# InternetMaximalism/plonky2_bn254

Measured on AMD Instinct MI355X. Metric: G1 scalar-mul STARK proofs/sec (256-bit scalars), higher is better.
Workload: dtype u64 (Goldilocks p = 2^64-2^32+1; BN254 Fq as 10x26-bit Montgomery limbs); 1 GPU; configs[1]: batch of 1024 G1 scalar-muls on 1 GPU per step = 8 proofs x 128 instances, 2^16 rows, W=781, standard_fast_config; instances_per_proof=128, steps_in_flight=4, parallelism=1 GPU, no collective

## Files before the change

### include/bn254_stark.h

```cpp
#ifndef BN254_STARK_H
#define BN254_STARK_H

#include <stddef.h>
#include <stdint.h>

#ifdef __cplusplus
extern "C" {
#endif

#define BN254S_ABI_VERSION 1

enum {
  BN254S_OK = 0,
  BN254S_E_INVALID_ARG = -1,
  BN254S_E_HIP = -2,
  BN254S_E_OOM = -3,
  BN254S_E_INVALID_POINT = -4,
  BN254S_E_UNSUPPORTED = -5,
  BN254S_E_TRANSCRIPT = -6,
  BN254S_E_INTERNAL = -7,
  BN254S_E_VERIFY = -8
};

typedef struct bn254s_ctx bn254s_ctx;
// ... 133 lines not shown
                       const uint64_t* offset, size_t n, size_t per_proof, uint64_t* outputs_out, bn254s_proof** proofs_out);
int bn254s_commit_values(bn254s_ctx* ctx, const uint64_t* values, size_t ncols, uint64_t* coeffs, uint64_t* lde,
                         uint64_t* cap);
int bn254s_bench_ntt(bn254s_ctx* ctx, size_t ncols, int iters, float* ms);
int bn254s_bench_ntt_clock(bn254s_ctx* ctx, size_t ncols, int iters, float* ms, float* mhz, float* mhz_min);
int bn254s_bench_issue(bn254s_ctx* ctx, float* ns_per_issue, float* mhz);
int bn254s_bench_copy(bn254s_ctx* ctx, size_t words, int iters);
int bn254s_bench_leafhash(bn254s_ctx* ctx, size_t ncols, int log_leaves, int iters, float* ms);
int bn254s_poseidon_permute(bn254s_ctx* ctx, uint64_t* states, size_t n);
int bn254s_selftest_field(bn254s_ctx* ctx, const uint64_t* a, const uint64_t* b, size_t n, uint64_t* out);
int bn254s_selftest_poseidon(bn254s_ctx* ctx, int variant, uint64_t* states, size_t n);
int bn254s_selftest_leaf_hash(bn254s_ctx* ctx, const uint64_t* data, size_t ncols, int log_leaves, int kernel, int chunk_cols,
                              uint64_t* digests);
int bn254s_selftest_fq_inv(bn254s_ctx* ctx, const uint64_t* x, size_t n, uint64_t* out);
int bn254s_selftest_fq(bn254s_ctx* ctx, int group, const uint64_t* in, size_t n, uint64_t* out);
int bn254s_generate_trace(bn254s_ctx* ctx, int kind, const uint64_t* scalars, const uint64_t* x, const uint64_t* offset,
                          size_t n, uint32_t min_rows_log2, uint64_t* trace_out, uint64_t* outputs);
int bn254s_g1_generate_trace(bn254s_ctx* ctx, const uint64_t* scalars, const uint64_t* x, const uint64_t* offset,
                             size_t n, uint32_t min_rows_log2, uint64_t* trace_out, uint64_t* outputs);

#ifdef __cplusplus
}
#endif
#endif
```

### plonky2_bn254_amd/csrc/aux.hip

```cpp
#include "aux.h"

static constexpr int LOGUP_CHUNK = 30;

__global__ __launch_bounds__(256) void k_logup_helpers(const u64* __restrict__ trace, size_t N, int rc_begin, int n_rc,
                                                       u64 beta0, u64 beta1, u64* __restrict__ aux, int helpers_per_ch,
                                                       u64* __restrict__ psum, int nchunks) {
  const size_t i = (size_t)blockIdx.x * blockDim.x + threadIdx.x;
  if (i >= N) return;
  const int chunk = blockIdx.y, ch = blockIdx.z;
  const u64 beta = ch ? beta1 : beta0;
  const int k0 = chunk * LOGUP_CHUNK;
  const int cnt = min(LOGUP_CHUNK, helpers_per_ch - k0);
  const u64* col = trace + (size_t)(rc_begin + 2 * k0) * N + i;
  u64 prod[LOGUP_CHUNK], pre[LOGUP_CHUNK];
  u64 acc = 1;
#pragma unroll
  for (int j = 0; j < LOGUP_CHUNK; j++) {
    if (j < cnt) {
      const u64 a = gl_add(col[(size_t)(2 * j) * N], beta);
      const bool two = 2 * (k0 + j) + 1 < n_rc;
      prod[j] = two ? gl_mul(a, gl_add(col[(size_t)(2 * j + 1) * N], beta)) : a;
      pre[j] = acc;
      acc = gl_mul(acc, prod[j]);
    }
  }
  u64 inv = gl_inv(acc);
  u64 sum = 0;
  const u64 beta2 = gl_dbl(beta);
  u64* out = aux + (size_t)ch * (helpers_per_ch + 1) * N + i;
#pragma unroll
  for (int j = LOGUP_CHUNK - 1; j >= 0; j--) {
    if (j < cnt) {
      u64 h = gl_mul(inv, pre[j]);
      inv = gl_mul(inv, prod[j]);
      if (2 * (k0 + j) + 1 < n_rc) h = gl_mul(h, gl_add(gl_add(col[(size_t)(2 * j) * N], col[(size_t)(2 * j + 1) * N]), beta2));
      out[(size_t)(k0 + j) * N] = h;
      sum = gl_add(sum, h);
    }
  }
  psum[(size_t)(ch * nchunks + chunk) * N + i] = sum;
}

__global__ __launch_bounds__(256) void k_logup_terms(const u64* __restrict__ trace, size_t N, int table_col, int freq_col,
                                                     u64 beta0, u64 beta1, const u64* __restrict__ psum, int nchunks,
                                                     u64* __restrict__ terms) {
  const size_t i = (size_t)blockIdx.x * blockDim.x + threadIdx.x;
  if (i >= N) return;
  const int ch = blockIdx.y;
  const u64 beta = ch ? beta1 : beta0;
  u64 s = 0;
  for (int c = 0; c < nchunks; c++) s = gl_add(s, psum[(size_t)(ch * nchunks + c) * N + i]);
  u64 t = gl_inv(gl_add(beta, trace[(size_t)table_col * N + i]));
  s = gl_sub(s, gl_mul(trace[(size_t)freq_col * N + i], t));
  terms[(size_t)ch * N + i] = s;
}

__global__ __launch_bounds__(1024) void k_scan(const u64* __restrict__ in, size_t in_stride, u64* __restrict__ out,
                                               size_t out_stride, size_t N, int mode) {
  LATENCY_KERNEL_PRIO();
  __shared__ u64 part[1024];
  const int t = threadIdx.x;
  const u64* src = in + (size_t)blockIdx.x * in_stride;
  u64* dst = out + (size_t)blockIdx.x * out_stride;
  const size_t per = N / 1024;
  auto idx = [&](size_t q) { return mode ? N - 1 - q : q; };
  size_t q0 = (size_t)t * per;
  u64 s = 0;
  for (size_t q = 0; q < per; q++) s = gl_add(s, src[idx(q0 + q)]);
  part[t] = s;
  __syncthreads();
  for (int off = 1; off < 1024; off <<= 1) {
    u64 v = t >= off ? part[t - off] : 0;
    __syncthreads();
    part[t] = gl_add(part[t], v);
    __syncthreads();
  }
  u64 run = t ? part[t - 1] : 0;
  for (size_t q = 0; q < per; q++) {
    u64 x = src[idx(q0 + q)];
    if (mode == 0) {
      dst[idx(q0 + q)] = run;
      run = gl_add(run, x);
    } else {
      run = gl_add(run, x);
      dst[idx(q0 + q)] = run;
    }
// ... 14 lines not shown
      int start = spec.col_start[ctl][m], nb = spec.col_bits[ctl][m];
      u64 v = 0;
      for (int b = nb - 1; b >= 0; b--) v = gl_add(gl_dbl(v), trace[(size_t)(start + b) * N + i]);
      a0 = gl_add(gl_mul(a0, beta0), v);
      a1 = gl_add(gl_mul(a1, beta1), v);
    }
    t0 = gl_inv(gl_add(a0, gamma0));
    t1 = gl_inv(gl_add(a1, gamma1));
  } else if (f != 0) {
    atomicCAS(err, 0, BN254S_E_INTERNAL);
  }
  terms[(size_t)(ctl * 2 + 0) * N + i] = t0;
  terms[(size_t)(ctl * 2 + 1) * N + i] = t1;
}

size_t aux_scratch_words(const StarkShape& sh, size_t N) {
  int nchunks = (sh.n_helpers() + LOGUP_CHUNK - 1) / LOGUP_CHUNK;
  return (size_t)(2 * nchunks + 2 + 2 * sh.n_ctl) * N;
}

void aux_build(const StarkShape& sh, const u64* d_trace, size_t N, const u64 betas[2], const u64 gammas[2], u64* d_aux,
               u64* d_scratch, int* d_err, hipStream_t st) {
  const int n_rc = sh.n_rc(), m = sh.n_helpers();
  const int nchunks = (m + LOGUP_CHUNK - 1) / LOGUP_CHUNK;
  u64* psum = d_scratch;
  u64* terms = psum + (size_t)2 * nchunks * N;
  u64* cterms = terms + 2 * N;
  dim3 g1((unsigned)((N + 255) / 256), nchunks, 2);
  k_logup_helpers<<<g1, 256, 0, st>>>(d_trace, N, sh.rc_begin, n_rc, betas[0], betas[1], d_aux, m, psum, nchunks);
  dim3 g2((unsigned)((N + 255) / 256), 2);
  k_logup_terms<<<g2, 256, 0, st>>>(d_trace, N, sh.table_col, sh.freq_col, betas[0], betas[1], psum, nchunks, terms);
  k_scan<<<2, 1024, 0, st>>>(terms, N, d_aux + (size_t)m * N, (size_t)(m + 1) * N, N, 0);
  dim3 g3((unsigned)((N + 255) / 256), sh.n_ctl);
  k_ctl_terms<<<g3, 256, 0, st>>>(d_trace, N, sh.ctl, betas[0], gammas[0], betas[1], gammas[1], cterms, d_err);
  k_scan<<<2 * sh.n_ctl, 1024, 0, st>>>(cterms, N, d_aux + (size_t)2 * (m + 1) * N, N, N, 1);
}

void aux_module_warm() {
  hipFuncAttributes a;
  (void)hipFuncGetAttributes(&a, reinterpret_cast<const void*>(&k_logup_terms));
}
```

### plonky2_bn254_amd/csrc/capi.hip

```cpp
#include <algorithm>
#include <cstring>
#include "ctx.h"
#include "merkle.h"
#include "trace_g1.h"
#include "fq_selftest.h"
#include "poseidon_dev.h"

void ntt_module_warm();
void merkle_module_warm();
void aux_module_warm();
void fri_module_warm();
void quotient_g1_module_warm();
void quotient_g2fq_module_warm();
void trace_g1_module_warm();
void trace_g2fq_module_warm();
void prover_module_warm();

extern "C" {

int bn254s_abi_version(void) { return BN254S_ABI_VERSION; }

void bn254s_params_default(bn254s_params* p) {
  p->struct_size = sizeof(bn254s_params);
  p->security_bits = 100;
// ... 448 lines not shown

int bn254s_selftest_fq_inv(bn254s_ctx* c, const uint64_t* x, size_t n, uint64_t* out) {
  if (!c || !x || !out) return BN254S_E_INVALID_ARG;
  if (n == 0) return BN254S_OK;
  HIP_TRY(c, hipSetDevice(c->device));
  u64* d = c->words("fi.io", 12 * n);
  if (!d) return BN254S_E_OOM;
  HIP_TRY(c, hipMemcpyAsync(d, x, 32 * n, hipMemcpyHostToDevice, c->stream));
  launch_fq_inv_selftest(d, d + 4 * n, n, c->stream);
  HIP_TRY(c, hipGetLastError());
  HIP_TRY(c, hipMemcpyAsync(out, d + 4 * n, 64 * n, hipMemcpyDeviceToHost, c->stream));
  HIP_TRY(c, hipStreamSynchronize(c->stream));
  return BN254S_OK;
}

static bool selftest_fq_below_p(const uint64_t* w) {
  static const uint64_t P[4] = {0x3c208c16d87cfd47ULL, 0x97816a916871ca8dULL, 0xb85045b68181585dULL, 0x30644e72e131a029ULL};
  for (int j = 3; j >= 0; j--)
    if (w[j] != P[j]) return w[j] < P[j];
  return false;
}
int bn254s_selftest_fq(bn254s_ctx* c, int group, const uint64_t* in, size_t n, uint64_t* out) {
  if (!c || !in || !out || group < 0 || group >= FQ_SELFTEST_GROUPS) return BN254S_E_INVALID_ARG;
  if (n == 0) return BN254S_OK;
  const size_t wi = (size_t)FQ_SELFTEST_IN[group], wo = (size_t)FQ_SELFTEST_OUT[group];
  auto is_zero = [](const uint64_t* w, int words) {
    uint64_t o = 0;
    for (int k = 0; k < words; k++) o |= w[k];
    return o == 0;
  };
// ... 21 lines not shown
```

### plonky2_bn254_amd/csrc/fri.h

```cpp
#pragma once
#include "quotient_common.h"

__host__ __device__ inline size_t merkle_level_offset_dev(int log_leaves, int level) {
  return ((size_t)2 << log_leaves) - ((size_t)2 << (log_leaves - level));
}

static constexpr size_t FRI_OPENING_ZQ_WORDS = 2 * 256 * 4, FRI_OPENING_TABLE_WORDS = 2 * FRI_OPENING_ZQ_WORDS;
void fri_opening_tables(unsigned log_r, gl2 zeta, gl2 zeta_next, u64* d_tables, hipStream_t st);
void fri_openings(const u64* d_coeffs, size_t N, unsigned log_r, int npolys, const u64* d_tables, u64* d_out, hipStream_t st);

void fri_combine(const StarkShape& sh, const u64* d_tl, const u64* d_al, const u64* d_ql, const u64* d_apow, const u64* d_xs,
                 gl2 zeta, gl2 zeta_next, gl2 r0, gl2 r1, gl2 r2, gl2 alpha, size_t M2, u64* d_out, hipStream_t st);

void fri_combine_coeffs(const StarkShape& sh, const u64* d_tcoef, const u64* d_acoef, const u64* d_qcoef, const u64* d_apow, size_t N,
                        u64* d_comb, hipStream_t st);
void fri_combine_final(const StarkShape& sh, const u64* d_comb_lde, const u64* d_xs, gl2 zeta, gl2 zeta_next, gl2 r0, gl2 r1, gl2 r2,
                       gl2 alpha, size_t M2, u64* d_out, hipStream_t st);
void fri_extract_window(const u64* d_lde, size_t M2, unsigned log_n, int h, size_t k0, size_t rows, int ncols, u64* d_out, hipStream_t st);
void fri_gather_rows(const u64* d_lde, size_t M2, int ncols, const u32* d_indices, int nq, u64* d_out, hipStream_t st);

void fri_fold(const u64* d_in, u64* d_out, unsigned log_m, u64 shift, gl2 beta, u64 inv16, hipStream_t st);

void fri_pow_launch(const u64 state[12], int pos, u64 base, unsigned pow_bits, size_t count, unsigned long long* d_result,
                    hipStream_t st);

static constexpr int FRI_MAX_LAYERS = 8;
struct QueryGatherArgs {
// ... 15 lines not shown
```

### plonky2_bn254_amd/csrc/fri.hip

```cpp
#include "fri.h"
#include "poseidon_dev.h"

static constexpr int OPEN_Q = (int)(65536 / 256);

__global__ __launch_bounds__(256) void k_opening_tables(gl2 z0r, gl2 z1r, u64* __restrict__ zq, u64* __restrict__ zt) {
  LATENCY_KERNEL_PRIO();
  const int t = threadIdx.x;
  u32* zq3 = reinterpret_cast<u32*>(zq);
  for (int pt = 0; pt < 2; pt++) {
    const gl2 z = pt ? z1r : z0r;
    gl2 a = gl2_pow(gl2_pow(z, 256), (u64)t), b = gl2_pow(z, (u64)t);
    const W3 a0 = w3_split(a.c0), a1 = w3_split(a.c1);
    u32* e = zq3 + (size_t)(pt * OPEN_Q + t) * 8;
    e[0] = a0.w0; e[1] = a0.w1; e[2] = a0.w2; e[3] = 0;
    e[4] = a1.w0; e[5] = a1.w1; e[6] = a1.w2; e[7] = 0;
    zt[(pt * 256 + t) * 2] = b.c0;
    zt[(pt * 256 + t) * 2 + 1] = b.c1;
  }
}

__global__ __launch_bounds__(256) void k_openings(const u64* __restrict__ coeffs, size_t N, unsigned log_r, const u64* __restrict__ zq,
                                                  const u64* __restrict__ zt, u64* __restrict__ out) {
  __shared__ u64 red[256 * 5];
  const int t = threadIdx.x;
// ... 51 lines not shown

struct CombineArgs {
  const u64* tl;
  const u64* al;
  const u64* ql;
  const u32* apow3;
  const u64* xs;
  int W, A, num_lookup;
  gl2 zeta, zeta_next;
  gl2 r0, r1, r2;
  gl2 a_n1n2, a_n2;
  u64* out;
  size_t M2;
};

__global__ __launch_bounds__(256) void k_fri_combine(CombineArgs A) {
  const size_t j = (size_t)blockIdx.x * blockDim.x + threadIdx.x;
  if (j >= A.M2) return;
  const size_t M2 = A.M2;
  Acc3 g0, g1, z0, z1, q0, q1;
  acc3_init(g0);
  acc3_init(g1);
  acc3_init(z0);
  acc3_init(z1);
  acc3_init(q0);
  acc3_init(q1);
  auto mad2 = [&](Acc3& a0, Acc3& a1, u64 v, const u32* e) {
    const u32 v0 = (u32)v & M22, v1 = (u32)(v >> 22) & M22, v2 = (u32)(v >> 44);
    acc3_mad(a0, v0, v1, v2, e[0], e[1], e[2]);
    acc3_mad(a1, v0, v1, v2, e[4], e[5], e[6]);
  };
#pragma unroll 8
  for (int c = 0; c < A.W; c++) mad2(g0, g1, A.tl[(size_t)c * M2 + j], A.apow3 + 8 * (size_t)c);
  const u32* ap = A.apow3 + 8 * (size_t)A.W;
#pragma unroll 8
  for (int c = 0; c < A.num_lookup; c++) mad2(g0, g1, A.al[(size_t)c * M2 + j], ap + 8 * (size_t)c);
  for (int c = A.num_lookup; c < A.A; c++) {
    u64 v = A.al[(size_t)c * M2 + j];
    mad2(g0, g1, v, ap + 8 * (size_t)c);
    mad2(z0, z1, v, A.apow3 + 8 * (size_t)(c - A.num_lookup));
  }
  gl2 f1 = gl2_make(acc3_red(g0), acc3_red(g1));
  ap = A.apow3 + 8 * (size_t)(A.W + A.A);
  for (int c = 0; c < 4; c++) mad2(q0, q1, A.ql[(size_t)c * M2 + j], ap + 8 * (size_t)c);
  gl2 f0 = gl2_add(f1, gl2_make(acc3_red(q0), acc3_red(q1)));
  gl2 f2 = gl2_make(acc3_red(z0), acc3_red(z1));
  const u64 x = A.xs[j];
  gl2 xe = gl2_make(x, 0);
  gl2 t0 = gl2_mul(gl2_sub(f0, A.r0), gl2_inv(gl2_sub(xe, A.zeta)));
  gl2 t1 = gl2_mul(gl2_sub(f1, A.r1), gl2_inv(gl2_sub(xe, A.zeta_next)));
  gl2 t2 = gl2_mul_base(gl2_sub(f2, A.r2), gl_inv(gl_sub(x, 1)));
  gl2 r = gl2_add(gl2_add(gl2_mul(t0, A.a_n1n2), gl2_mul(t1, A.a_n2)), t2);
  reinterpret_cast<ulonglong2*>(A.out)[j] = make_ulonglong2(r.c0, r.c1);
}

__global__ __launch_bounds__(256) void k_fri_combine_coeffs(CombineArgs A, u64* __restrict__ comb) {
  const size_t j = (size_t)blockIdx.x * blockDim.x + threadIdx.x;
  if (j >= A.M2) return;
  const size_t M2 = A.M2;
  Acc3 g0, g1, z0, z1, q0, q1;
  acc3_init(g0);
  acc3_init(g1);
  acc3_init(z0);
  acc3_init(z1);
  acc3_init(q0);
  acc3_init(q1);
  auto mad2 = [&](Acc3& a0, Acc3& a1, u64 v, const u32* e) {
    const u32 v0 = (u32)v & M22, v1 = (u32)(v >> 22) & M22, v2 = (u32)(v >> 44);
    acc3_mad(a0, v0, v1, v2, e[0], e[1], e[2]);
    acc3_mad(a1, v0, v1, v2, e[4], e[5], e[6]);
// ... 5 lines not shown
  for (int c = 0; c < A.num_lookup; c++) mad2(g0, g1, A.al[(size_t)c * M2 + j], ap + 8 * (size_t)c);
  for (int c = A.num_lookup; c < A.A; c++) {
    u64 v = A.al[(size_t)c * M2 + j];
    mad2(g0, g1, v, ap + 8 * (size_t)c);
    mad2(z0, z1, v, A.apow3 + 8 * (size_t)(c - A.num_lookup));
  }
  ap = A.apow3 + 8 * (size_t)(A.W + A.A);
  for (int c = 0; c < 4; c++) mad2(q0, q1, A.ql[(size_t)c * M2 + j], ap + 8 * (size_t)c);
  comb[0 * M2 + j] = acc3_red(g0);
  comb[1 * M2 + j] = acc3_red(g1);
  comb[2 * M2 + j] = acc3_red(q0);
  comb[3 * M2 + j] = acc3_red(q1);
  comb[4 * M2 + j] = acc3_red(z0);
  comb[5 * M2 + j] = acc3_red(z1);
}
__global__ __launch_bounds__(256) void k_fri_combine_final(CombineArgs A, const u64* __restrict__ cl ) {
  const size_t j = (size_t)blockIdx.x * blockDim.x + threadIdx.x;
  if (j >= A.M2) return;
  const size_t M2 = A.M2;
  const gl2 f1 = gl2_make(cl[0 * M2 + j], cl[1 * M2 + j]);
  const gl2 f0 = gl2_add(f1, gl2_make(cl[2 * M2 + j], cl[3 * M2 + j]));
  const gl2 f2 = gl2_make(cl[4 * M2 + j], cl[5 * M2 + j]);
  const u64 x = A.xs[j];
  gl2 xe = gl2_make(x, 0);
  gl2 t0 = gl2_mul(gl2_sub(f0, A.r0), gl2_inv(gl2_sub(xe, A.zeta)));
  gl2 t1 = gl2_mul(gl2_sub(f1, A.r1), gl2_inv(gl2_sub(xe, A.zeta_next)));
  gl2 t2 = gl2_mul_base(gl2_sub(f2, A.r2), gl_inv(gl_sub(x, 1)));
  gl2 r = gl2_add(gl2_add(gl2_mul(t0, A.a_n1n2), gl2_mul(t1, A.a_n2)), t2);
  reinterpret_cast<ulonglong2*>(A.out)[j] = make_ulonglong2(r.c0, r.c1);
}
static CombineArgs combine_args(const StarkShape& sh, const u64* d_tl, const u64* d_al, const u64* d_ql, const u64* d_apow, const u64* d_xs,
                                gl2 zeta, gl2 zeta_next, gl2 r0, gl2 r1, gl2 r2, gl2 alpha, size_t M2, u64* d_out) {
  CombineArgs A;
  A.tl = d_tl;
  A.al = d_al;
  A.ql = d_ql;
  A.apow3 = reinterpret_cast<const u32*>(d_apow);
  A.xs = d_xs;
  A.W = sh.W;
  A.A = sh.n_aux();
  A.num_lookup = sh.n_lookup_cols();
  A.zeta = zeta;
// ... 28 lines not shown
  const u32 k = (u32)((k0 + t) & (N - 1));
  out[(size_t)blockIdx.y * rows + t] = lde[(size_t)blockIdx.y * M2 + ((size_t)h << log_n) + bitrev32(k, log_n)];
}
void fri_extract_window(const u64* d_lde, size_t M2, unsigned log_n, int h, size_t k0, size_t rows, int ncols, u64* d_out, hipStream_t st) {
  k_extract_window<<<dim3((unsigned)((rows + 255) / 256), ncols), 256, 0, st>>>(d_lde, M2, log_n, (u32)h, k0, rows, d_out);
}
__global__ void k_gather_rows(const u64* __restrict__ lde, size_t M2, const u32* __restrict__ indices, int nq, u64* __restrict__ out) {
  const int q = blockIdx.x * blockDim.x + threadIdx.x;
  if (q >= nq) return;
  out[(size_t)blockIdx.y * nq + q] = lde[(size_t)blockIdx.y * M2 + indices[q]];
}
void fri_gather_rows(const u64* d_lde, size_t M2, int ncols, const u32* d_indices, int nq, u64* d_out, hipStream_t st) {
  k_gather_rows<<<dim3((unsigned)((nq + 63) / 64), ncols), 64, 0, st>>>(d_lde, M2, d_indices, nq, d_out);
}

void fri_combine(const StarkShape& sh, const u64* d_tl, const u64* d_al, const u64* d_ql, const u64* d_apow, const u64* d_xs,
                 gl2 zeta, gl2 zeta_next, gl2 r0, gl2 r1, gl2 r2, gl2 alpha, size_t M2, u64* d_out, hipStream_t st) {
  CombineArgs A = combine_args(sh, d_tl, d_al, d_ql, d_apow, d_xs, zeta, zeta_next, r0, r1, r2, alpha, M2, d_out);
  k_fri_combine<<<(unsigned)((M2 + 255) / 256), 256, 0, st>>>(A);
}

template <int E>
__device__ __forceinline__ u64 mul_w16inv(u64 x) {
  if constexpr (E == 0) return x;
  else return gl_mul_2exp<192 - 12 * E>(x);
}
template <int SPAN, int G, int J>
__device__ __forceinline__ void ibfly(u64* x) {
  constexpr int E = J * (8 / SPAN);
  u64 a = x[G + J], b = x[G + J + SPAN];
  x[G + J] = gl_add(a, b);
  if constexpr (E == 0) x[G + J + SPAN] = gl_sub(a, b);
  else x[G + J + SPAN] = gl_mul_2exp<96 - 12 * E>(gl_sub(b, a));
}
__device__ __forceinline__ void idft16(u64* x) {
#define BF(SPAN, G, J) ibfly<SPAN, G, J>(x)
// ... 124 lines not shown
```

### plonky2_bn254_amd/csrc/prover.hip

```cpp
#include <algorithm>
#include <atomic>
#include <cstring>
#include <thread>
#include "ctx.h"
#include "trace_g1.h"
#include "trace_g2fq.h"
#include "aux.h"
#include "merkle.h"
#include "quotient.h"
#include "fri.h"
#include "transcript.h"
#include "prover.h"

template <class L>
static StarkShape make_shape(bool input_has_a, int n_constraints) {
  StarkShape s;
  s.W = L::W;
  s.rc_begin = L::RC_BEGIN;
  s.rc_end = L::RC_END;
  s.table_col = L::RANGE;
  s.freq_col = L::FREQ;
  s.n_ctl = 2;
  s.n_constraints = n_constraints;
  memset(&s.ctl, 0, sizeof(s.ctl));
// ... 270 lines not shown
  }
  u64* d_in = mem.words("in", in_words + 16);
  u64* d_tvals = mem.words("tvals", lowmem && !stream ? std::max((size_t)W * N, (size_t)A * M2) : (size_t)W * N);
  u64* d_tcoef = mem.words("tcoef", (size_t)W * N);
  u64* d_hist = mem.words("hist", 65536 / 2);
  u64* d_tmp = mem.words("tmp", log_s ? (size_t)3 * CH * N : lowmem ? (size_t)CH * N : (size_t)(log_r ? 1 : 3) * std::max(W, A) * N);
  d_tmp_fwd = d_tmp;
  mem.drop("win");
  if (stream) {
    mem.drop("tlde");
    mem.drop("alde");
    mem.drop("acoef");
  } else {
    mem.drop("ldechunk");
    mem.drop("sponge");
    mem.drop("comb");
  }
  u64* d_ldechunk = stream ? mem.words("ldechunk", (size_t)CH * M2) : nullptr;
  u64* d_sponge = stream ? mem.words("sponge", (size_t)12 * M2) : nullptr;
  u64* d_comb = stream ? mem.words("comb", (size_t)6 * N + (size_t)6 * M2) : nullptr;
  u64* d_tlde = stream ? d_ldechunk : mem.words("tlde", (size_t)W * M2);
  const size_t tree_words = merkle_tree_digests(log_m2, P.cap_height) * 4;
  u64* d_trees = mem.words("trees", 3 * tree_words);
  u64* d_avals = mem.words("avals", (size_t)A * N);
  u64* d_acoef = lowmem ? d_avals : mem.words("acoef", (size_t)A * N);
  u64* d_alde = stream ? d_ldechunk : lowmem ? d_tvals : mem.words("alde", (size_t)A * M2);
  const size_t trace_scr = kind == KIND_G1 ? g1_trace_scratch_words(n) : kind == KIND_G2 ? g2_trace_scratch_words(n) : fq_trace_scratch_words(n);
  u64* d_scr = mem.words("scratch", std::max(trace_scr, aux_scratch_words(sh, N)));
  u64* d_q = mem.words("quot", (size_t)(3 * NQ) * N + (size_t)NQ * M2 + (size_t)QUOTIENT_MAX_PARTS * 2 * (stream ? WROWS : M2));
  u64* d_tabs = mem.words("tabs", QUOTIENT_W_WORDS(K) + QUOTIENT_MZT_WORDS + 4 * (size_t)(W + A + NQ));
  u64* d_open = mem.words("open", std::max((size_t)(W + A + NQ) * NSPL * R * 5 + FRI_OPENING_TABLE_WORDS, n * (size_t)PW));
  size_t fri_words = 0, fri_tree_words = 0;
  {
    size_t m = M2;
    for (int l = 0; l <= L; l++) {
// ... 12 lines not shown
      wpq += 32 + 4 * (lg - P.cap_height);
    }
  }
  u64* d_qout = mem.words("qout", wpq * P.num_queries + 64);
  {
    const size_t need = std::max((size_t)(W + A + NQ) * NSPL * R * 5, wpq * P.num_queries) * 8;
    if (sl.pinned_bytes < need) {
      if (sl.pinned) hipHostFree(sl.pinned);
      sl.pinned = nullptr;
      sl.pinned_bytes = 0;
      CHK(hipHostMalloc(&sl.pinned, need));
      sl.pinned_bytes = need;
    }
  }
  if (!d_hist || !d_in || !d_tvals || !d_tcoef || !d_tmp || !d_tlde || !d_trees || !d_avals || !d_acoef || !d_alde || !d_scr || !d_q ||
      !d_tabs || !d_open || !d_fri || !d_fritrees || !d_qout || (stream && (!d_ldechunk || !d_sponge || !d_comb))) {
    err = mem.err;
    mem.release();
    return BN254S_E_OOM;
  }
  {
    static const size_t reserve = (size_t)(getenv("BN254S_MEM_RESERVE_MB") ? atol(getenv("BN254S_MEM_RESERVE_MB")) : 6144) << 20;
    size_t free_b = 0, total_b = 0;
    if (hipMemGetInfo(&free_b, &total_b) == hipSuccess && free_b < reserve) {
      err = "device memory: " + std::to_string(free_b >> 20) + " MB would be left free, below the reserve of " +
            std::to_string(reserve >> 20) + " MB kept for the runtime's own allocations";
      mem.release();
      return BN254S_E_OOM;
    }
  }
  if (after_alloc) (*after_alloc)();
// ... 271 lines not shown
    gl2 ap = gl2_make(1, 0), r0 = gl2_make(0, 0), r1 = r0, r2 = r0;
    for (int p = 0; p < W + A + NQ; p++) {
      const W3 s0 = w3_split(ap.c0), s1 = w3_split(ap.c1);
      u32* e = &apow[8 * (size_t)p];
      e[0] = s0.w0; e[1] = s0.w1; e[2] = s0.w2;
      e[4] = s1.w0; e[5] = s1.w1; e[6] = s1.w2;
      r0 = gl2_add(r0, gl2_mul(ap, gl2_make(op(p, 0), op(p, 1))));
      if (p < W + A) r1 = gl2_add(r1, gl2_mul(ap, gl2_make(op(p, 2), op(p, 3))));
      if (p < n_ctlz) r2 = gl2_add(r2, gl2_mul_base(ap, op(W + num_lookup + p, 4)));
      ap = gl2_mul(ap, fri_alpha);
    }
    CHK(hipMemcpyAsync(d_apow, apow.data(), apow.size() * 4, hipMemcpyHostToDevice, st));
    CHK(hipStreamSynchronize(st));
    BigSection big(c, st, BIG_EXCL);
    sb(ST_FRI);
    if (stream) {
      fri_combine_coeffs(sh, d_tcoef, d_acoef, d_qcoef, d_apow, N, d_comb, st);
      do_lde(d_comb, d_comb + (size_t)6 * N, 6);
      fri_combine_final(sh, d_comb + (size_t)6 * N, pt.x, zeta, zeta_next, r0, r1, r2, fri_alpha, M2, d_fri, st);
    } else {
      fri_combine(sh, d_tlde, d_alde, d_qlde, d_apow, pt.x, zeta, zeta_next, r0, r1, r2, fri_alpha, M2, d_fri, st);
    }
  }
  std::vector<std::vector<u64>> layer_caps(L, std::vector<u64>(CAPW));
  std::vector<const u64*> layer_vals(L), layer_trees(L);
  u64* vals = d_fri;
  u64* ftree = d_fritrees;
  u64 shift = GL_GEN;
  unsigned lm = log_m2;
  const u64 inv16 = gl_inv(16);
  for (int l = 0; l < L; l++) {
    const int lg = (int)lm - 4;
    merkle_build(vals, 32, 1, 32, lg, P.cap_height, ftree, st, mmode());
    CHK(hipMemcpyAsync(layer_caps[l].data(), ftree + 4 * merkle_level_offset(lg, lg - P.cap_height), CAPW * 8,
                       hipMemcpyDeviceToHost, st));
    CHK(hipStreamSynchronize(st));
    ch.observe_n(layer_caps[l].data(), CAPW);
// ... 429 lines not shown
```

### plonky2_bn254_amd/lib.py

```python
from __future__ import annotations

import ctypes as C
import os
from typing import Optional

import numpy as np

_HERE = os.path.dirname(os.path.abspath(__file__))
LIB_PATH = os.environ.get("BN254S_LIB") or os.path.join(_HERE, "libbn254stark.so")

U64P = C.POINTER(C.c_uint64)


class LibraryMissing(RuntimeError):
    pass


class VerifyError(RuntimeError):
    """bn254s_verify rejected the proof; the message is the reference verifier's error text."""


class Params(C.Structure):
    _fields_ = [(n, C.c_uint32) for n in (
        "struct_size", "security_bits", "num_challenges", "rate_bits", "cap_height", "pow_bits",
# ... 62 lines not shown
    lib.bn254s_hash_to_g2_batch.argtypes = [vp, vp, C.c_size_t, C.c_size_t, vp]
    lib.bn254s_job_outputs_batch.argtypes = [vp, C.c_int, vp, vp, vp, C.c_size_t, vp, vp]
    lib.bn254s_job_outputs.argtypes = [vp, C.c_int, C.POINTER(Params), vp, vp, vp, C.c_size_t, C.c_size_t, vp, C.POINTER(vp)]
    lib.bn254s_hash_to_fq2_batch.argtypes = [vp, vp, C.c_size_t, C.c_size_t, vp]
    lib.bn254s_ctl_values.argtypes = [C.c_int, vp, vp, vp, vp, C.c_size_t, vp, vp]
    lib.bn254s_commit_values.argtypes = [vp, vp, C.c_size_t, vp, vp, vp]
    lib.bn254s_bench_ntt.argtypes = [vp, C.c_size_t, C.c_int, C.POINTER(C.c_float)]
    lib.bn254s_bench_ntt_clock.argtypes = [vp, C.c_size_t, C.c_int, C.POINTER(C.c_float), C.POINTER(C.c_float), C.POINTER(C.c_float)]
    lib.bn254s_bench_issue.argtypes = [vp, C.POINTER(C.c_float), C.POINTER(C.c_float)]
    lib.bn254s_poseidon_permute.argtypes = [vp, vp, C.c_size_t]
    lib.bn254s_selftest_field.argtypes = [vp, vp, vp, C.c_size_t, vp]
    lib.bn254s_selftest_poseidon.argtypes = [vp, C.c_int, vp, C.c_size_t]
    lib.bn254s_selftest_leaf_hash.argtypes = [vp, vp, C.c_size_t, C.c_int, C.c_int, C.c_int, vp]
    lib.bn254s_selftest_fq_inv.argtypes = [vp, vp, C.c_size_t, vp]
    lib.bn254s_selftest_fq.argtypes = [vp, C.c_int, vp, C.c_size_t, vp]
    lib.bn254s_bench_copy.argtypes = [vp, C.c_size_t, C.c_int]
    lib.bn254s_bench_leafhash.argtypes = [vp, C.c_size_t, C.c_int, C.c_int, C.POINTER(C.c_float)]
    lib.bn254s_g1_generate_trace.argtypes = [vp, vp, vp, vp, C.c_size_t, C.c_uint32, vp, vp]
    _lib = lib
    return lib


def default_params() -> Params:
    p = Params()
    load_library().bn254s_params_default(C.byref(p))
    return p


def _ptr(a: Optional[np.ndarray]):
    if a is None:
# ... 411 lines not shown
        x = np.ascontiguousarray(x, dtype=np.uint64)
        out = np.zeros((x.shape[0], 8), np.uint64)
        self._check(self._lib.bn254s_selftest_fq_inv(self._h, _ptr(x), x.shape[0], _ptr(out)), "bn254s_selftest_fq_inv")
        return out

    SELFTEST_FQ_WORDS = ((16, 68), (16, 60), (32, 92), (72, 74))

    def selftest_fq(self, group: int, rows: np.ndarray) -> np.ndarray:
        rows = np.ascontiguousarray(rows, dtype=np.uint64)
        if not 0 <= group < len(self.SELFTEST_FQ_WORDS):
            raise ValueError(f"selftest_fq: unknown group {group}")
        wi, wo = self.SELFTEST_FQ_WORDS[group]
        assert rows.ndim == 2 and rows.shape[1] == wi, (rows.shape, wi)
        out = np.zeros((rows.shape[0], wo), np.uint64)
        self._check(self._lib.bn254s_selftest_fq(self._h, group, _ptr(rows), rows.shape[0], _ptr(out)), "bn254s_selftest_fq")
        return out

    def poseidon_permute(self, states: np.ndarray) -> np.ndarray:
        st = np.ascontiguousarray(states, dtype=np.uint64).copy()
        self._check(self._lib.bn254s_poseidon_permute(self._h, _ptr(st), st.shape[0]), "bn254s_poseidon_permute")
        return st

    def generate_trace(self, kind, scalars, x, offset=None, min_rows_log2=16):
        width, pw = {0: (781, 8), 1: (1295, 16), 2: (427, 4)}[kind]
        n = scalars.shape[0]
        rows = max(1 << min_rows_log2, 512 * n)
        rows = 1 << (rows - 1).bit_length()
        trace = np.zeros((width, rows), np.uint64)
        outs = np.zeros((n, pw), np.uint64)
        self._check(self._lib.bn254s_generate_trace(self._h, kind, _ptr(scalars), _ptr(x), _ptr(offset), n, min_rows_log2,
# ... 368 lines not shown
```

Baseline: 90.47 proofs/s.

## Replace per-row LogUp inversions with precomputed 16-bit inverse table lookups

LogUp helper columns are now built from a precomputed table of 1/(beta+v) for every 16-bit v and both challenges, built once per proof with small batched inversions. This replaces the per-row batch inversion and extra multiplies, and handles both challenges in one pass over the trace. Values of 65536 or more are flagged through the error word rather than computed. The FRI combine-final kernel now uses one shared inversion of the quadratic-extension norms instead of three separate inversions. The non-streaming FRI combine path is removed so the coefficient-LDE path always runs, which costs an always-allocated comb buffer. A selftest entry point for LogUp is also added.

```diff
diff --git a/include/bn254_stark.h b/include/bn254_stark.h
--- a/include/bn254_stark.h
+++ b/include/bn254_stark.h
@@ -171,6 +171,8 @@
                               uint64_t* digests);
 int bn254s_selftest_fq_inv(bn254s_ctx* ctx, const uint64_t* x, size_t n, uint64_t* out);
 int bn254s_selftest_fq(bn254s_ctx* ctx, int group, const uint64_t* in, size_t n, uint64_t* out);
+int bn254s_selftest_logup(bn254s_ctx* ctx, const uint64_t* trace, size_t rows, int ncols, int rc_begin, int n_rc, int table_col,
+                          int freq_col, const uint64_t betas[2], uint64_t* out);
 int bn254s_generate_trace(bn254s_ctx* ctx, int kind, const uint64_t* scalars, const uint64_t* x, const uint64_t* offset,
                           size_t n, uint32_t min_rows_log2, uint64_t* trace_out, uint64_t* outputs);
 int bn254s_g1_generate_trace(bn254s_ctx* ctx, const uint64_t* scalars, const uint64_t* x, const uint64_t* offset,
diff --git a/plonky2_bn254_amd/csrc/aux.hip b/plonky2_bn254_amd/csrc/aux.hip
--- a/plonky2_bn254_amd/csrc/aux.hip
+++ b/plonky2_bn254_amd/csrc/aux.hip
@@ -1,58 +1,93 @@
+#include <algorithm>
 #include "aux.h"
 
-static constexpr int LOGUP_CHUNK = 30;
+static constexpr int LOGUP_SPAN = 16;
+static constexpr int LOGUP_INV_BATCH = 4;
+
+__global__ __launch_bounds__(256) void k_logup_inv_table(u64 beta0, u64 beta1, u64* __restrict__ inv) {
+  const u32 t = blockIdx.x * blockDim.x + threadIdx.x;
+  if (t >= 2 * 65536 / LOGUP_INV_BATCH) return;
+  u64 d[LOGUP_INV_BATCH], pre[LOGUP_INV_BATCH];
+  u64 acc = 1;
+#pragma unroll
+  for (int j = 0; j < LOGUP_INV_BATCH; j++) {
+    const u64 x = gl_add((j & 1) ? beta1 : beta0, (u64)(2 * t + (j >> 1)));
+    d[j] = x ? x : 1;
+    pre[j] = acc;
+    acc = gl_mul(acc, d[j]);
+  }
+  u64 r = gl_inv(acc);
+  u64 o[LOGUP_INV_BATCH];
+#pragma unroll
+  for (int j = LOGUP_INV_BATCH - 1; j >= 0; j--) {
+    const u64 x = gl_add((j & 1) ? beta1 : beta0, (u64)(2 * t + (j >> 1)));
+    o[j] = x ? gl_mul(r, pre[j]) : 0;
+    r = gl_mul(r, d[j]);
+  }
+  ulonglong2* out = reinterpret_cast<ulonglong2*>(inv) + 2 * (size_t)t;
+  out[0] = make_ulonglong2(o[0], o[1]);
+  out[1] = make_ulonglong2(o[2], o[3]);
+}
+
+__device__ __forceinline__ ulonglong2 logup_inv_at(const ulonglong2* __restrict__ inv, u64 v, u64& bad) {
+  bad |= v;
+  return inv[(u32)v & 0xFFFFu];
+}
 
 __global__ __launch_bounds__(256) void k_logup_helpers(const u64* __restrict__ trace, size_t N, int rc_begin, int n_rc,
-                                                       u64 beta0, u64 beta1, u64* __restrict__ aux, int helpers_per_ch,
-                                                       u64* __restrict__ psum, int nchunks) {
+                                                       const u64* __restrict__ inv_tab, u64* __restrict__ aux, int helpers_per_ch,
+                                                       u64* __restrict__ psum, int nchunks, int* __restrict__ err) {
   const size_t i = (size_t)blockIdx.x * blockDim.x + threadIdx.x;
   if (i >= N) return;
-  const int chunk = blockIdx.y, ch = blockIdx.z;
-  const u64 beta = ch ? beta1 : beta0;
-  const int k0 = chunk * LOGUP_CHUNK;
-  const int cnt = min(LOGUP_CHUNK, helpers_per_ch - k0);
+  const ulonglong2* inv = reinterpret_cast<const ulonglong2*>(inv_tab);
+  const int chunk = blockIdx.y;
+  const int k0 = chunk * LOGUP_SPAN;
+  const int k1 = min(k0 + LOGUP_SPAN, helpers_per_ch);
+  const int kp = min(k1, n_rc / 2);
   const u64* col = trace + (size_t)(rc_begin + 2 * k0) * N + i;
-  u64 prod[LOGUP_CHUNK], pre[LOGUP_CHUNK];
-  u64 acc = 1;
-#pragma unroll
-  for (int j = 0; j < LOGUP_CHUNK; j++) {
-    if (j < cnt) {
-      const u64 a = gl_add(col[(size_t)(2 * j) * N], beta);
-      const bool two = 2 * (k0 + j) + 1 < n_rc;
-      prod[j] = two ? gl_mul(a, gl_add(col[(size_t)(2 * j + 1) * N], beta)) : a;
-      pre[j] = acc;
-      acc = gl_mul(acc, prod[j]);
-    }
+  u64* out0 = aux + (size_t)k0 * N + i;
+  u64* out1 = out0 + (size_t)(helpers_per_ch + 1) * N;
+  u64 s0 = 0, s1 = 0, bad = 0;
+#pragma unroll 4
+  for (int k = k0; k < kp; k++) {
+    const ulonglong2 ia = logup_inv_at(inv, col[0], bad), ib = logup_inv_at(inv, col[N], bad);
+    const u64 h0 = gl_add(ia.x, ib.x), h1 = gl_add(ia.y, ib.y);
+    *out0 = h0;
+    *out1 = h1;
+    s0 = gl_add(s0, h0);
+    s1 = gl_add(s1, h1);
+    col += 2 * N;
+    out0 += N;
+    out1 += N;
   }
-  u64 inv = gl_inv(acc);
-  u64 sum = 0;
-  const u64 beta2 = gl_dbl(beta);
-  u64* out = aux + (size_t)ch * (helpers_per_ch + 1) * N + i;
-#pragma unroll
-  for (int j = LOGUP_CHUNK - 1; j >= 0; j--) {
-    if (j < cnt) {
-      u64 h = gl_mul(inv, pre[j]);
-      inv = gl_mul(inv, prod[j]);
-      if (2 * (k0 + j) + 1 < n_rc) h = gl_mul(h, gl_add(gl_add(col[(size_t)(2 * j) * N], col[(size_t)(2 * j + 1) * N]), beta2));
-      out[(size_t)(k0 + j) * N] = h;
-      sum = gl_add(sum, h);
-    }
+  if (kp < k1) {
+    const ulonglong2 ia = logup_inv_at(inv, col[0], bad);
+    *out0 = ia.x;
+    *out1 = ia.y;
+    s0 = gl_add(s0, ia.x);
+    s1 = gl_add(s1, ia.y);
   }
-  psum[(size_t)(ch * nchunks + chunk) * N + i] = sum;
+  psum[(size_t)chunk * N + i] = s0;
+  psum[(size_t)(nchunks + chunk) * N + i] = s1;
+  if (bad >> 16) atomicCAS(err, 0, BN254S_E_INTERNAL);
 }
 
 __global__ __launch_bounds__(256) void k_logup_terms(const u64* __restrict__ trace, size_t N, int table_col, int freq_col,
-                                                     u64 beta0, u64 beta1, const u64* __restrict__ psum, int nchunks,
-                                                     u64* __restrict__ terms) {
+                                                     const u64* __restrict__ inv_tab, const u64* __restrict__ psum, int nchunks,
+                                                     u64* __restrict__ terms, int* __restrict__ err) {
   const size_t i = (size_t)blockIdx.x * blockDim.x + threadIdx.x;
   if (i >= N) return;
-  const int ch = blockIdx.y;
-  const u64 beta = ch ? beta1 : beta0;
-  u64 s = 0;
-  for (int c = 0; c < nchunks; c++) s = gl_add(s, psum[(size_t)(ch * nchunks + c) * N + i]);
-  u64 t = gl_inv(gl_add(beta, trace[(size_t)table_col * N + i]));
-  s = gl_sub(s, gl_mul(trace[(size_t)freq_col * N + i], t));
-  terms[(size_t)ch * N + i] = s;
+  u64 bad = 0;
+  const ulonglong2 t = logup_inv_at(reinterpret_cast<const ulonglong2*>(inv_tab), trace[(size_t)table_col * N + i], bad);
+  const u64 f = trace[(size_t)freq_col * N + i];
+  u64 s0 = 0, s1 = 0;
+  for (int c = 0; c < nchunks; c++) {
+    s0 = gl_add(s0, psum[(size_t)c * N + i]);
+    s1 = gl_add(s1, psum[(size_t)(nchunks + c) * N + i]);
+  }
+  terms[i] = gl_sub(s0, gl_mul(f, t.x));
+  terms[N + i] = gl_sub(s1, gl_mul(f, t.y));
+  if (bad >> 16) atomicCAS(err, 0, BN254S_E_INTERNAL);
 }
 
 __global__ __launch_bounds__(1024) void k_scan(const u64* __restrict__ in, size_t in_stride, u64* __restrict__ out,
@@ -62,14 +97,15 @@
   const int t = threadIdx.x;
   const u64* src = in + (size_t)blockIdx.x * in_stride;
   u64* dst = out + (size_t)blockIdx.x * out_stride;
-  const size_t per = N / 1024;
+  const int T = blockDim.x;
+  const size_t per = N / T;
   auto idx = [&](size_t q) { return mode ? N - 1 - q : q; };
   size_t q0 = (size_t)t * per;
   u64 s = 0;
   for (size_t q = 0; q < per; q++) s = gl_add(s, src[idx(q0 + q)]);
   part[t] = s;
   __syncthreads();
-  for (int off = 1; off < 1024; off <<= 1) {
+  for (int off = 1; off < T; off <<= 1) {
     u64 v = t >= off ? part[t - off] : 0;
     __syncthreads();
     part[t] = gl_add(part[t], v);
@@ -114,26 +150,30 @@
   terms[(size_t)(ctl * 2 + 1) * N + i] = t1;
 }
 
+static constexpr size_t LOGUP_INV_WORDS = 2 * 65536;
 size_t aux_scratch_words(const StarkShape& sh, size_t N) {
-  int nchunks = (sh.n_helpers() + LOGUP_CHUNK - 1) / LOGUP_CHUNK;
-  return (size_t)(2 * nchunks + 2 + 2 * sh.n_ctl) * N;
+  int nchunks = (sh.n_helpers() + LOGUP_SPAN - 1) / LOGUP_SPAN;
+  return LOGUP_INV_WORDS + (size_t)(2 * nchunks + 2 + 2 * sh.n_ctl) * N;
 }
 
 void aux_build(const StarkShape& sh, const u64* d_trace, size_t N, const u64 betas[2], const u64 gammas[2], u64* d_aux,
                u64* d_scratch, int* d_err, hipStream_t st) {
   const int n_rc = sh.n_rc(), m = sh.n_helpers();
-  const int nchunks = (m + LOGUP_CHUNK - 1) / LOGUP_CHUNK;
-  u64* psum = d_scratch;
+  const int nchunks = (m + LOGUP_SPAN - 1) / LOGUP_SPAN;
+  u64* inv = d_scratch;
+  u64* psum = inv + LOGUP_INV_WORDS;
   u64* terms = psum + (size_t)2 * nchunks * N;
   u64* cterms = terms + 2 * N;
-  dim3 g1((unsigned)((N + 255) / 256), nchunks, 2);
-  k_logup_helpers<<<g1, 256, 0, st>>>(d_trace, N, sh.rc_begin, n_rc, betas[0], betas[1], d_aux, m, psum, nchunks);
-  dim3 g2((unsigned)((N + 255) / 256), 2);
-  k_logup_terms<<<g2, 256, 0, st>>>(d_trace, N, sh.table_col, sh.freq_col, betas[0], betas[1], psum, nchunks, terms);
-  k_scan<<<2, 1024, 0, st>>>(terms, N, d_aux + (size_t)m * N, (size_t)(m + 1) * N, N, 0);
+  const unsigned scan_threads = (unsigned)std::min<size_t>(1024, N);
+  k_logup_inv_table<<<(unsigned)(LOGUP_INV_WORDS / LOGUP_INV_BATCH / 256), 256, 0, st>>>(betas[0], betas[1], inv);
+  dim3 g1((unsigned)((N + 255) / 256), nchunks);
+  k_logup_helpers<<<g1, 256, 0, st>>>(d_trace, N, sh.rc_begin, n_rc, inv, d_aux, m, psum, nchunks, d_err);
+  k_logup_terms<<<(unsigned)((N + 255) / 256), 256, 0, st>>>(d_trace, N, sh.table_col, sh.freq_col, inv, psum, nchunks, terms, d_err);
+  k_scan<<<2, scan_threads, 0, st>>>(terms, N, d_aux + (size_t)m * N, (size_t)(m + 1) * N, N, 0);
+  if (sh.n_ctl == 0) return;
   dim3 g3((unsigned)((N + 255) / 256), sh.n_ctl);
   k_ctl_terms<<<g3, 256, 0, st>>>(d_trace, N, sh.ctl, betas[0], gammas[0], betas[1], gammas[1], cterms, d_err);
-  k_scan<<<2 * sh.n_ctl, 1024, 0, st>>>(cterms, N, d_aux + (size_t)2 * (m + 1) * N, N, N, 1);
+  k_scan<<<2 * sh.n_ctl, scan_threads, 0, st>>>(cterms, N, d_aux + (size_t)2 * (m + 1) * N, N, N, 1);
 }
 
 void aux_module_warm() {
diff --git a/plonky2_bn254_amd/csrc/capi.hip b/plonky2_bn254_amd/csrc/capi.hip
--- a/plonky2_bn254_amd/csrc/capi.hip
+++ b/plonky2_bn254_amd/csrc/capi.hip
@@ -4,6 +4,7 @@
 #include "merkle.h"
 #include "trace_g1.h"
 #include "fq_selftest.h"
+#include "aux.h"
 #include "poseidon_dev.h"
 
 void ntt_module_warm();
@@ -486,6 +487,46 @@
   return BN254S_OK;
 }
 
+int bn254s_selftest_logup(bn254s_ctx* c, const uint64_t* trace, size_t rows, int ncols, int rc_begin, int n_rc, int table_col,
+                          int freq_col, const uint64_t betas[2], uint64_t* out) {
+  if (!c || !trace || !betas || !out) return BN254S_E_INVALID_ARG;
+  if (rows < 64 || rows > ((size_t)1 << 20) || (rows & (rows - 1)) || ncols < 1 || ncols > 4096 || n_rc < 1 || rc_begin < 0 ||
+      rc_begin > ncols - n_rc || table_col < 0 || table_col >= ncols || freq_col < 0 || freq_col >= ncols)
+    return BN254S_E_INVALID_ARG;
+  if (betas[0] >= GL_P || betas[1] >= GL_P) return BN254S_E_INVALID_ARG;
+  for (size_t k = 0; k < (size_t)ncols * rows; k++)
+    if (trace[k] >= GL_P) return BN254S_E_INVALID_ARG;
+  StarkShape sh;
+  sh.W = ncols;
+  sh.rc_begin = rc_begin;
+  sh.rc_end = rc_begin + n_rc;
+  sh.table_col = table_col;
+  sh.freq_col = freq_col;
+  sh.n_ctl = 0;
+  memset(&sh.ctl, 0, sizeof(sh.ctl));
+  const size_t tw = (size_t)ncols * rows, aw = (size_t)sh.n_lookup_cols() * rows;
+  HIP_TRY(c, hipSetDevice(c->device));
+  u64* d = c->words("lu.io", tw + aw + aux_scratch_words(sh, rows) + 2);
+  if (!d) return BN254S_E_OOM;
+  u64* d_aux = d + tw;
+  u64* d_scr = d_aux + aw;
+  int* d_err = (int*)(d_scr + aux_scratch_words(sh, rows));
+  const u64 gammas[2] = {0, 0};
+  int h_err = 0;
+  HIP_TRY(c, hipMemcpyAsync(d, trace, 8 * tw, hipMemcpyHostToDevice, c->stream));
+  HIP_TRY(c, hipMemsetAsync(d_err, 0, 8, c->stream));
+  aux_build(sh, d, rows, betas, gammas, d_aux, d_scr, d_err, c->stream);
+  HIP_TRY(c, hipGetLastError());
+  HIP_TRY(c, hipMemcpyAsync(out, d_aux, 8 * aw, hipMemcpyDeviceToHost, c->stream));
+  HIP_TRY(c, hipMemcpyAsync(&h_err, d_err, 4, hipMemcpyDeviceToHost, c->stream));
+  HIP_TRY(c, hipStreamSynchronize(c->stream));
+  if (h_err) {
+    c->set_err("LogUp columns: device error " + std::to_string(h_err) + " (a range-checked or table value above 65535)");
+    return h_err;
+  }
+  return BN254S_OK;
+}
+
 static bool selftest_fq_below_p(const uint64_t* w) {
   static const uint64_t P[4] = {0x3c208c16d87cfd47ULL, 0x97816a916871ca8dULL, 0xb85045b68181585dULL, 0x30644e72e131a029ULL};
   for (int j = 3; j >= 0; j--)
diff --git a/plonky2_bn254_amd/csrc/fri.h b/plonky2_bn254_amd/csrc/fri.h
--- a/plonky2_bn254_amd/csrc/fri.h
+++ b/plonky2_bn254_amd/csrc/fri.h
@@ -8,9 +8,6 @@
 static constexpr size_t FRI_OPENING_ZQ_WORDS = 2 * 256 * 4, FRI_OPENING_TABLE_WORDS = 2 * FRI_OPENING_ZQ_WORDS;
 void fri_opening_tables(unsigned log_r, gl2 zeta, gl2 zeta_next, u64* d_tables, hipStream_t st);
 void fri_openings(const u64* d_coeffs, size_t N, unsigned log_r, int npolys, const u64* d_tables, u64* d_out, hipStream_t st);
-
-void fri_combine(const StarkShape& sh, const u64* d_tl, const u64* d_al, const u64* d_ql, const u64* d_apow, const u64* d_xs,
-                 gl2 zeta, gl2 zeta_next, gl2 r0, gl2 r1, gl2 r2, gl2 alpha, size_t M2, u64* d_out, hipStream_t st);
 
 void fri_combine_coeffs(const StarkShape& sh, const u64* d_tcoef, const u64* d_acoef, const u64* d_qcoef, const u64* d_apow, size_t N,
                         u64* d_comb, hipStream_t st);
diff --git a/plonky2_bn254_amd/csrc/fri.hip b/plonky2_bn254_amd/csrc/fri.hip
--- a/plonky2_bn254_amd/csrc/fri.hip
+++ b/plonky2_bn254_amd/csrc/fri.hip
@@ -89,46 +89,6 @@
   size_t M2;
 };
 
-__global__ __launch_bounds__(256) void k_fri_combine(CombineArgs A) {
-  const size_t j = (size_t)blockIdx.x * blockDim.x + threadIdx.x;
-  if (j >= A.M2) return;
-  const size_t M2 = A.M2;
-  Acc3 g0, g1, z0, z1, q0, q1;
-  acc3_init(g0);
-  acc3_init(g1);
-  acc3_init(z0);
-  acc3_init(z1);
-  acc3_init(q0);
-  acc3_init(q1);
-  auto mad2 = [&](Acc3& a0, Acc3& a1, u64 v, const u32* e) {
-    const u32 v0 = (u32)v & M22, v1 = (u32)(v >> 22) & M22, v2 = (u32)(v >> 44);
-    acc3_mad(a0, v0, v1, v2, e[0], e[1], e[2]);
-    acc3_mad(a1, v0, v1, v2, e[4], e[5], e[6]);
-  };
-#pragma unroll 8
-  for (int c = 0; c < A.W; c++) mad2(g0, g1, A.tl[(size_t)c * M2 + j], A.apow3 + 8 * (size_t)c);
-  const u32* ap = A.apow3 + 8 * (size_t)A.W;
-#pragma unroll 8
-  for (int c = 0; c < A.num_lookup; c++) mad2(g0, g1, A.al[(size_t)c * M2 + j], ap + 8 * (size_t)c);
-  for (int c = A.num_lookup; c < A.A; c++) {
-    u64 v = A.al[(size_t)c * M2 + j];
-    mad2(g0, g1, v, ap + 8 * (size_t)c);
-    mad2(z0, z1, v, A.apow3 + 8 * (size_t)(c - A.num_lookup));
-  }
-  gl2 f1 = gl2_make(acc3_red(g0), acc3_red(g1));
-  ap = A.apow3 + 8 * (size_t)(A.W + A.A);
-  for (int c = 0; c < 4; c++) mad2(q0, q1, A.ql[(size_t)c * M2 + j], ap + 8 * (size_t)c);
-  gl2 f0 = gl2_add(f1, gl2_make(acc3_red(q0), acc3_red(q1)));
-  gl2 f2 = gl2_make(acc3_red(z0), acc3_red(z1));
-  const u64 x = A.xs[j];
-  gl2 xe = gl2_make(x, 0);
-  gl2 t0 = gl2_mul(gl2_sub(f0, A.r0), gl2_inv(gl2_sub(xe, A.zeta)));
-  gl2 t1 = gl2_mul(gl2_sub(f1, A.r1), gl2_inv(gl2_sub(xe, A.zeta_next)));
-  gl2 t2 = gl2_mul_base(gl2_sub(f2, A.r2), gl_inv(gl_sub(x, 1)));
-  gl2 r = gl2_add(gl2_add(gl2_mul(t0, A.a_n1n2), gl2_mul(t1, A.a_n2)), t2);
-  reinterpret_cast<ulonglong2*>(A.out)[j] = make_ulonglong2(r.c0, r.c1);
-}
-
 __global__ __launch_bounds__(256) void k_fri_combine_coeffs(CombineArgs A, u64* __restrict__ comb) {
   const size_t j = (size_t)blockIdx.x * blockDim.x + threadIdx.x;
   if (j >= A.M2) return;
@@ -164,6 +124,11 @@
   comb[4 * M2 + j] = acc3_red(z0);
   comb[5 * M2 + j] = acc3_red(z1);
 }
+__device__ __forceinline__ u64 gl2_norm(gl2 a) {
+  const u64 t = gl_mul(a.c1, a.c1);
+  const u64 t7 = gl_add(gl_add(gl_dbl(gl_dbl(t)), gl_dbl(t)), t);
+  return gl_sub(gl_mul(a.c0, a.c0), t7);
+}
 __global__ __launch_bounds__(256) void k_fri_combine_final(CombineArgs A, const u64* __restrict__ cl ) {
   const size_t j = (size_t)blockIdx.x * blockDim.x + threadIdx.x;
   if (j >= A.M2) return;
@@ -173,9 +138,17 @@
   const gl2 f2 = gl2_make(cl[4 * M2 + j], cl[5 * M2 + j]);
   const u64 x = A.xs[j];
   gl2 xe = gl2_make(x, 0);
-  gl2 t0 = gl2_mul(gl2_sub(f0, A.r0), gl2_inv(gl2_sub(xe, A.zeta)));
-  gl2 t1 = gl2_mul(gl2_sub(f1, A.r1), gl2_inv(gl2_sub(xe, A.zeta_next)));
-  gl2 t2 = gl2_mul_base(gl2_sub(f2, A.r2), gl_inv(gl_sub(x, 1)));
+  const gl2 d0 = gl2_sub(xe, A.zeta), d1 = gl2_sub(xe, A.zeta_next);
+  const u64 n0 = gl2_norm(d0), n1 = gl2_norm(d1), n2 = gl_sub(x, 1);
+  const u64 m0 = n0 ? n0 : 1, m1 = n1 ? n1 : 1, m2 = n2 ? n2 : 1;
+  const u64 m01 = gl_mul(m0, m1);
+  u64 ri = gl_inv(gl_mul(m01, m2));
+  const u64 i2 = n2 ? gl_mul(ri, m01) : 0;
+  ri = gl_mul(ri, m2);
+  const u64 i0 = n0 ? gl_mul(ri, m1) : 0, i1 = n1 ? gl_mul(ri, m0) : 0;
+  gl2 t0 = gl2_mul(gl2_sub(f0, A.r0), gl2_make(gl_mul(d0.c0, i0), gl_mul(gl_neg(d0.c1), i0)));
+  gl2 t1 = gl2_mul(gl2_sub(f1, A.r1), gl2_make(gl_mul(d1.c0, i1), gl_mul(gl_neg(d1.c1), i1)));
+  gl2 t2 = gl2_mul_base(gl2_sub(f2, A.r2), i2);
   gl2 r = gl2_add(gl2_add(gl2_mul(t0, A.a_n1n2), gl2_mul(t1, A.a_n2)), t2);
   reinterpret_cast<ulonglong2*>(A.out)[j] = make_ulonglong2(r.c0, r.c1);
 }
@@ -234,12 +207,6 @@
   k_gather_rows<<<dim3((unsigned)((nq + 63) / 64), ncols), 64, 0, st>>>(d_lde, M2, d_indices, nq, d_out);
 }
 
-void fri_combine(const StarkShape& sh, const u64* d_tl, const u64* d_al, const u64* d_ql, const u64* d_apow, const u64* d_xs,
-                 gl2 zeta, gl2 zeta_next, gl2 r0, gl2 r1, gl2 r2, gl2 alpha, size_t M2, u64* d_out, hipStream_t st) {
-  CombineArgs A = combine_args(sh, d_tl, d_al, d_ql, d_apow, d_xs, zeta, zeta_next, r0, r1, r2, alpha, M2, d_out);
-  k_fri_combine<<<(unsigned)((M2 + 255) / 256), 256, 0, st>>>(A);
-}
-
 template <int E>
 __device__ __forceinline__ u64 mul_w16inv(u64 x) {
   if constexpr (E == 0) return x;
diff --git a/plonky2_bn254_amd/csrc/prover.hip b/plonky2_bn254_amd/csrc/prover.hip
--- a/plonky2_bn254_amd/csrc/prover.hip
+++ b/plonky2_bn254_amd/csrc/prover.hip
@@ -308,11 +308,10 @@
   } else {
     mem.drop("ldechunk");
     mem.drop("sponge");
-    mem.drop("comb");
   }
   u64* d_ldechunk = stream ? mem.words("ldechunk", (size_t)CH * M2) : nullptr;
   u64* d_sponge = stream ? mem.words("sponge", (size_t)12 * M2) : nullptr;
-  u64* d_comb = stream ? mem.words("comb", (size_t)6 * N + (size_t)6 * M2) : nullptr;
+  u64* d_comb = mem.words("comb", (size_t)6 * N + (size_t)6 * M2);
   u64* d_tlde = stream ? d_ldechunk : mem.words("tlde", (size_t)W * M2);
   const size_t tree_words = merkle_tree_digests(log_m2, P.cap_height) * 4;
   u64* d_trees = mem.words("trees", 3 * tree_words);
@@ -355,7 +354,7 @@
     }
   }
   if (!d_hist || !d_in || !d_tvals || !d_tcoef || !d_tmp || !d_tlde || !d_trees || !d_avals || !d_acoef || !d_alde || !d_scr || !d_q ||
-      !d_tabs || !d_open || !d_fri || !d_fritrees || !d_qout || (stream && (!d_ldechunk || !d_sponge || !d_comb))) {
+      !d_tabs || !d_open || !d_fri || !d_fritrees || !d_qout || !d_comb || (stream && (!d_ldechunk || !d_sponge))) {
     err = mem.err;
     mem.release();
     return BN254S_E_OOM;
@@ -657,13 +656,9 @@
     CHK(hipStreamSynchronize(st));
     BigSection big(c, st, BIG_EXCL);
     sb(ST_FRI);
-    if (stream) {
-      fri_combine_coeffs(sh, d_tcoef, d_acoef, d_qcoef, d_apow, N, d_comb, st);
-      do_lde(d_comb, d_comb + (size_t)6 * N, 6);
-      fri_combine_final(sh, d_comb + (size_t)6 * N, pt.x, zeta, zeta_next, r0, r1, r2, fri_alpha, M2, d_fri, st);
-    } else {
-      fri_combine(sh, d_tlde, d_alde, d_qlde, d_apow, pt.x, zeta, zeta_next, r0, r1, r2, fri_alpha, M2, d_fri, st);
-    }
+    fri_combine_coeffs(sh, d_tcoef, d_acoef, d_qcoef, d_apow, N, d_comb, st);
+    do_lde(d_comb, d_comb + (size_t)6 * N, 6);
+    fri_combine_final(sh, d_comb + (size_t)6 * N, pt.x, zeta, zeta_next, r0, r1, r2, fri_alpha, M2, d_fri, st);
   }
   std::vector<std::vector<u64>> layer_caps(L, std::vector<u64>(CAPW));
   std::vector<const u64*> layer_vals(L), layer_trees(L);
diff --git a/plonky2_bn254_amd/lib.py b/plonky2_bn254_amd/lib.py
--- a/plonky2_bn254_amd/lib.py
+++ b/plonky2_bn254_amd/lib.py
@@ -100,6 +100,8 @@
     lib.bn254s_selftest_leaf_hash.argtypes = [vp, vp, C.c_size_t, C.c_int, C.c_int, C.c_int, vp]
     lib.bn254s_selftest_fq_inv.argtypes = [vp, vp, C.c_size_t, vp]
     lib.bn254s_selftest_fq.argtypes = [vp, C.c_int, vp, C.c_size_t, vp]
+    if hasattr(lib, "bn254s_selftest_logup"):
+        lib.bn254s_selftest_logup.argtypes = [vp, vp, C.c_size_t, C.c_int, C.c_int, C.c_int, C.c_int, C.c_int, vp, vp]
     lib.bn254s_bench_copy.argtypes = [vp, C.c_size_t, C.c_int]
     lib.bn254s_bench_leafhash.argtypes = [vp, C.c_size_t, C.c_int, C.c_int, C.POINTER(C.c_float)]
     lib.bn254s_g1_generate_trace.argtypes = [vp, vp, vp, vp, C.c_size_t, C.c_uint32, vp, vp]
@@ -541,6 +543,16 @@
         assert rows.ndim == 2 and rows.shape[1] == wi, (rows.shape, wi)
         out = np.zeros((rows.shape[0], wo), np.uint64)
         self._check(self._lib.bn254s_selftest_fq(self._h, group, _ptr(rows), rows.shape[0], _ptr(out)), "bn254s_selftest_fq")
+        return out
+
+    def selftest_logup(self, trace: np.ndarray, rc_begin: int, n_rc: int, table_col: int, freq_col: int, betas) -> np.ndarray:
+        trace = np.ascontiguousarray(trace, dtype=np.uint64)
+        assert trace.ndim == 2
+        ncols, rows = trace.shape
+        b = np.array([int(betas[0]), int(betas[1])], dtype=np.uint64)
+        out = np.zeros((2 * ((n_rc + 1) // 2 + 1), rows), np.uint64)
+        self._check(self._lib.bn254s_selftest_logup(self._h, _ptr(trace), rows, ncols, rc_begin, n_rc, table_col, freq_col, _ptr(b),
+                                                    _ptr(out)), "bn254s_selftest_logup")
         return out
 
     def poseidon_permute(self, states: np.ndarray) -> np.ndarray:
```

Result: faster. 91.84 proofs/s, median of 6 (+1.5%).
